# slcs-jsc/jurassic-gpu

Hardware: AMD Instinct MI355X
Metric: rays/s (radiance spectra/s) for limb EGA forward model (higher is better)
Workload: dtype f64; 1 GPU; limb_1e6; rays_total=1000000, channels=4, emitters=5, tables=synthetic 33p x 10T x ~203u per (gas, channel), fp32

## Files before the change

include/jurassic_hip.h:

```cpp
#ifndef JURASSIC_HIP_H
#define JURASSIC_HIP_H

#include "jurassic_abi.h"

#ifdef __cplusplus
extern "C" {
#endif

void formod(ctl_t const *ctl, atm_t *atm, obs_t *obs);
void formod_GPU(ctl_t const *ctl, atm_t *atm, obs_t *obs);
void formod_pencil(ctl_t const *ctl, atm_t *atm, obs_t *obs, int const ir);
void formod_contrib(ctl_t const *ctl, atm_t *atm, obs_t *obs, obs_t *contrib);
void formod_fov(ctl_t const *ctl, obs_t *obs);

void intpol_atm(ctl_t *ctl, atm_t *atm_dest, atm_t *atm_src);

typedef struct { size_t size1, size2, tda; double *data; void *block; int owner; } jur_gsl_matrix_t;
void kernel(ctl_t const *ctl, atm_t *atm, obs_t *obs, jur_gsl_matrix_t *k);

enum {
  JUR_OK = 0,
  JUR_EINVAL = -1,
  JUR_EIO = -2,
  JUR_ENOMEM = -3,
// ... 70 lines not shown
                   int n, double const *dz, double const *w);

int  jur_fov_apply_device(jur_model_t *m, long nr, double const *d_time, double const *d_vpz, double *d_rad,
                          double *d_tau, int n, double const *dz, double const *w, void *stream);

int  jur_intpol_atm(ctl_t const *ctl, atm_t *dest, atm_t const *src, int device);

int  jur_model_reserve(jur_model_t *m, long nr);

long jur_model_workspace_bytes(jur_model_t const *m);
int  jur_model_chunk_rays(jur_model_t const *m);
long jur_model_table_bytes(jur_model_t const *m);
int  jur_device_info(int device, char *pci_bus_id, int len, size_t *free_bytes, size_t *total_bytes);
int  jur_model_set_chunk_rays(jur_model_t *m, int rays);
int  jur_model_set_sort_rays(jur_model_t *m, int on);
int  jur_model_set_trace_multiple(jur_model_t *m, int mult);
int  jur_model_set_compact_workspace(jur_model_t *m, int on);
long jur_model_last_launches(jur_model_t const *m);
int  jur_model_set_workspace_budget(jur_model_t *m, long bytes);

int  jur_model_set_pencil(jur_model_t *m, long max_rays, int rays_per_group);
void jur_tune_trace(int lanes_per_ray);
void jur_tune_combine(int channels_per_group, int sync_segments, long min_lanes);

enum { JUR_ARITH_FAST = 0, JUR_ARITH_EXACT = 1 };
int  jur_model_set_arithmetic(jur_model_t *m, int mode);
int  jur_model_arithmetic(jur_model_t const *m);

int  jur_dropin_finalize(void);

int  jur_model_enable_timing(jur_model_t *m, int on);
int  jur_model_last_kernel_ms(jur_model_t *m, double out_ms[3], long out_launches[3]);
int  jur_model_last_pencil_ms(jur_model_t *m, double *out_ms, long *out_launches);
int  jur_model_last_contrib_ms(jur_model_t *m, double *out_ms, long *out_launches);

int jur_kat_ega_eps(jur_model_t *m, int ig, int id, long n, double const *tau, double const *t, double const *u,
                    double const *p, int mode, int chain, double *out);
int jur_kat_continua(jur_model_t *m, int id, long n, double const *p, double const *t, double const *q,
                     double const *u_co2, double const *u_h2o, double *out);
int jur_kat_update(jur_model_t *m, int id, long n, int what, double const *a, double const *b, double const *c,
                   double *rad, double *tau, double *src);
int jur_kat_traceray(jur_model_t *m, long nr, double const *const geom[7], double *los, double *tsurf, double *const tp[3],
                     int *np_out);

#ifdef __cplusplus
}
// ... 3 lines not shown
```

jurassic-gpu_amd/csrc/jur_internal.h:

```cpp
#ifndef JUR_INTERNAL_H
#define JUR_INTERNAL_H

#include <stdint.h>
#include "jurassic_hip.h"

#ifdef __cplusplus
extern "C" {
#endif

typedef struct { int a, b; } jur_int2;
typedef struct { float u, eps; } jur_ue_t;
typedef struct { float u0, e0, u1, e1; double du_de, de_du; } __attribute__((aligned(32))) jur_rec_t;
typedef struct { double p; int nt; int c0; } jur_lvl_t;
typedef struct { double t; int nu; int e0; } jur_crv_t;

typedef struct {
  double nu;
  double co2_cw296, co2_cw260, co2_cw230;
  double h2o_sc;
  double h2o_ratio;
  double h2o_lnr_hi, h2o_lnr_lo;
  double h2o_ctwfrn;
  double n2_b, n2_beta;
  double o2_b, o2_beta;
// ... 32 lines not shown

typedef struct {
  int n;
  int stride;
  int stride_eps;
  long first;
  int const *order;
  double const *geom[7];
  double *tp[3];
  double *rad, *tau;
  int *np_out;
  int *np;
  double *tsurf;
  double *los;
  double *eps;
  int const *eps_off;
  int *status;
} jur_chunk_t;

int jurk_prepare_atm(jur_view_t const *v, double *d_pslope, void *stream);
int jurk_launch_trace(jur_view_t const *v, jur_chunk_t const *c, void *stream);
int jurk_launch_ega(jur_view_t const *v, jur_chunk_t const *c, void *stream);
int jurk_launch_combine(jur_view_t const *v, jur_chunk_t const *c, void *stream);
int jurk_launch_contrib(jur_view_t const *v, jur_chunk_t const *c, long nr, double *rad_c, double *tau_c, void *stream);
int jurk_tile_max(int n, int const *d_np, int *d_tile_np, void *stream);
int jurk_launch_kquot(long nq, long n, double const *d_rad, double const *d_h, double *d_kq, void *stream);
void jurk_tune_combine(int group, int sync, long min_lanes);
void jurk_tune_trace(int lanes);
int jurk_launch_cg(jur_view_t const *v, jur_chunk_t const *c, double *cgp, double *cgt, double *cgu, void *stream);
int jurk_fill_records(jur_ue_t const *ue, jur_rec_t *rec, long long n, void *stream);
long jurk_sort_tmp_bytes(long nr);
int jurk_sort_rays(jur_view_t const *v, int by_profile, long nr, double const *d_geom, long ld, int *d_order, void *tmp,
                   long tmp_bytes, void *stream);

long jurk_pencil_lds_bytes(jur_view_t const *v, int RB);
int jurk_launch_pencil(jur_view_t const *v, jur_chunk_t const *c, int RB, void *stream);

int jurk_launch_fov(long nr, int nd, double const *time, double const *vpz, double const *rad0, double const *tau0, double *rad,
                    double *tau, long ld, int n, double const *dz, double const *w, int *status, void *stream);

int jurk_launch_intpol(int ip, int ng, int nw, int ns, int nd_, int nx, double cx, double cz, double const *src, double const *x1,
                       int const *idx, int const *nz, double const *dst, double const *x0, double *out, void *stream);

int jurk_kat_ega(jur_view_t const *v, int g, int d, long n, double const *tau, double const *t, double const *u, double const *p,
                 int mode, int chain, double *out, void *stream);
int jurk_kat_continua(jur_view_t const *v, int d, long n, double const *p, double const *t, double const *q, double const *u_co2,
// ... 113 lines not shown
```

jurassic-gpu_amd/csrc/jur_kernels.hip:

```cpp

#include <hip/hip_runtime.h>
#include <hipcub/hipcub.hpp>
#include <cstdlib>
#include <mutex>
#include "jur_internal.h"

#define NLOS JUR_NLOS
#define TBLNS JUR_TBLNS

namespace {

__device__ __forceinline__ double c01(double x) { return (x > 1.) ? 1. : ((x < 0.) ? 0. : x); }
__device__ __forceinline__ double c01_num(double x) { return __builtin_fmax(__builtin_fmin(x, 1.), 0.); }

__device__ __forceinline__ double lip(double x0, double y0, double x1, double y1, double x) {
  return y0 + (x - x0) * (y1 - y0) / (x1 - x0);
}

__device__ __forceinline__ double div_rcp(double a, double b, double r) {
  double const q = a * r;
  return __builtin_fma(__builtin_fma(-b, q, a), r, q);
}
__device__ __forceinline__ double lip_rcp(double x0, double y0, double x1, double y1, double x, double r) {
  return y0 + div_rcp((x - x0) * (y1 - y0), x1 - x0, r);
// ... 1055 lines not shown
  in.p = ldg<double>(row + JUR_F_P * 64, lane);
  in.t = ldg<double>(row + JUR_F_T * 64, lane);
  in.ds = ldg<double>(row + JUR_F_DS * 64, lane);
  in.k = ldg<double>(row + (size_t)f_k * 64, lane);
  in.u_co2 = ldg<double>(row + (size_t)f_co2 * 64, lane);
  in.q_h2o = ldg<double>(row + JUR_F_QH2O * 64, lane);
  in.u_h2o = ldg<double>(row + (size_t)f_h2o * 64, lane);
  double tg[8];
#pragma unroll
  for (int k = 0; k < 8; k++) tg[k] = (k < ng && ((has_table >> k) & 1u)) ? ld_stream(trow + (size_t)k * 64, lane) : 1.0;
  double pcur = 1.0;
#pragma unroll
  for (int k = 0; k < 8; k++) pcur *= tg[k];
  for (int g0 = 8; g0 < ng; g0 += 8) {
#pragma unroll
    for (int k = 0; k < 8; k++) tg[k] = (g0 + k < ng && g0 + k < 32 && ((has_table >> (g0 + k)) & 1u)) ? ld_stream(trow + (size_t)(g0 + k) * 64, lane) : 1.0;
#pragma unroll
    for (int k = 0; k < 8; k++) pcur *= tg[k];
  }
  in.pcur = pcur;
  return in;
}

__global__ __launch_bounds__(256, 6) void jur_combine_kernel(jur_view_t v, jur_chunk_t c, int nrb) {
  int const nd = v.nd, ng = v.ng;
  BlockItem const bi = xcd_block_item((int)blockIdx.x, nrb, nd);
  int const rb = bi.rb, d = bi.item;
  if (rb < 0) return;
  int const r = rb * blockDim.x + threadIdx.x;
  double *const sr = reinterpret_cast<double *>(jur_lds);
  Exp2Lds const e2t{sr + TBLNS};
  {
    double const *const gsr = v.sr + (size_t)d * TBLNS;
    for (int i = threadIdx.x; i < TBLNS; i += blockDim.x) sr[i] = gsr[i];
    if (threadIdx.x < 64) sr[TBLNS + threadIdx.x] = JUR_EXP2_64[threadIdx.x];
    __syncthreads();
  }
  if (r >= c.n) return;
  long const ray = c.order ? (long)c.order[r] : c.first + r;
  int const nfield = JUR_F_K + v.nw + ng;
  int const tile = __builtin_amdgcn_readfirstlane(r >> 6);
  unsigned const lane = (unsigned)(r & 63);
  size_t const R = (size_t)nfield * 64, Re = (size_t)nd * ng * 64;
  double const *const los = c.los + (size_t)tile * los_tile_doubles(nfield);
  double const *const epsb = c.eps + eps_tile_point0(c, tile) * Re + (size_t)d * ng * 64;
  jur_chan_t const ch = v.chan[d];
  int const f_k = JUR_F_K + ch.window, f_u = JUR_F_K + v.nw;
  bool const do_co2 = (v.fourbit & 8) && ch.co2_on, do_h2o = (v.fourbit & 4) && ch.h2o_on,
             do_n2 = (v.fourbit & 2) && ch.n2_on, do_o2 = (v.fourbit & 1) && ch.o2_on;
  size_t const oidx = (size_t)ray * nd + d;
  bool const masked = !isfinite(c.rad[oidx]);
  double rad = 0.0, tau = 1.0, pprev = 1.0;
  int const np = c.np[r];
  unsigned has_table = 0;
  for (int g = 0; g < ng && g < 32; g++) has_table |= (v.pair[g * nd + d].a >= 2 ? 1u : 0u) << g;
  int const f_co2 = do_co2 ? f_u + v.ig_co2 : JUR_F_P, f_h2o = do_h2o ? f_u + v.ig_h2o : JUR_F_P;
  for (int ip = 0; ip < np; ++ip) {
    SegmentIn const in = load_segment(los + (size_t)ip * R, epsb + (size_t)ip * Re, lane, f_k, f_co2, f_h2o, ng, has_table);
    double beta_ds = in.k * in.ds;
    if (do_co2) beta_ds += ctm_co2(ch, in.p, in.t, in.u_co2);
    double const rt = rcp_t(in.t);
    if (do_h2o) beta_ds += ctm_h2o(e2t, ch, in.p, in.t, rt, in.q_h2o, in.u_h2o);
    if (do_n2) beta_ds += ctm_n2(e2t, ch, in.p, in.t, rt) * in.ds;
    if (do_o2) beta_ds += ctm_o2(e2t, ch, in.p, in.t, rt) * in.ds;
    double const tau_gas = segment_tau_gas(in.pcur, pprev);
    pprev = in.pcur;
    new_obs_step(e2t, tau_gas, beta_ds, planck_src(sr, in.t), rad, tau);
  }
  ray_epilogue(sr, ch.nu, c.tsurf[r], v.write_bbt, rad, tau);
  if (masked) rad = __builtin_nan("");
  c.rad[oidx] = rad;
  c.tau[oidx] = tau;
}

#ifndef JUR_COMBINE_WAVES
#define JUR_COMBINE_WAVES 8
#endif
__global__ __launch_bounds__(512, JUR_COMBINE_WAVES) void jur_combine_group_kernel(jur_view_t v, jur_chunk_t c, int nsb, int CG, int SYNC) {
  int const nd = v.nd, ng = v.ng;
  int const ncg = (nd + CG - 1) / CG, SUB = (int)(blockDim.x >> 6) / CG;
  BlockItem const bi = xcd_block_item((int)blockIdx.x, nsb, ncg);
  int const sb = bi.rb, cg = bi.item;
  if (sb < 0) return;
  int const w = __builtin_amdgcn_readfirstlane((int)(threadIdx.x >> 6)), lane = (int)(threadIdx.x & 63);
  int const cw = w % CG, sub = w / CG;
  int const d = cg * CG + cw;
  bool const live_wave = d < nd;
  double *const sr = reinterpret_cast<double *>(jur_lds) + (size_t)cw * TBLNS;
  int *const npmax_sh = reinterpret_cast<int *>(reinterpret_cast<double *>(jur_lds) + (size_t)CG * TBLNS);
  Exp2Lds const e2t{reinterpret_cast<double *>(jur_lds) + (size_t)CG * TBLNS + 2};
  if (threadIdx.x == 0) *npmax_sh = 0;
  if (threadIdx.x < 64) reinterpret_cast<double *>(jur_lds)[(size_t)CG * TBLNS + 2 + threadIdx.x] = JUR_EXP2_64[threadIdx.x];
  for (int k = 0; k < CG; k++) {
    if (cg * CG + k >= nd) break;
    double const *const gsr = v.sr + (size_t)(cg * CG + k) * TBLNS;
// ... 764 lines not shown
  if (c->n <= 0) return 0;
  int const block = 64;
  static int const env_lanes = getenv("JUR_TRACE_LANES") ? atoi(getenv("JUR_TRACE_LANES")) : 0;
  int const forced = g_trace_lanes ? g_trace_lanes : env_lanes;
  int const lanes = forced == 1 || forced == 4 ? forced : ((c->n <= 65536 && v->ng >= 3) ? 4 : 1);
  int const grid = (int)(((long)c->n * lanes + block - 1) / block);
  if (lanes == 4) hipLaunchKernelGGL(jur_trace_lanes_kernel<4>, dim3(grid), dim3(block), 0, (hipStream_t)stream, *v, *c);
  else hipLaunchKernelGGL(jur_trace_kernel, dim3(grid), dim3(block), 0, (hipStream_t)stream, *v, *c);
  return (int)hipGetLastError();
}

static int raise_lds_limit(std::mutex &mu, unsigned long long &raised, void const *const *funcs, int nfunc, bool needed) {
  int dev = 0;
  if (hipGetDevice(&dev) != hipSuccess || dev < 0 || dev > 63) return (int)hipErrorInvalidDevice;
  std::lock_guard<std::mutex> lock(mu);
  if ((raised >> dev) & 1ull) return 0;
  hipError_t e = hipSuccess;
  for (int i = 0; i < nfunc && e == hipSuccess; i++) e = hipFuncSetAttribute(funcs[i], hipFuncAttributeMaxDynamicSharedMemorySize, 128 * 1024);
  if (e != hipSuccess) { (void)hipGetLastError(); return needed ? (int)e : 0; }
  raised |= 1ull << dev;
  return 0;
}

extern "C" int jurk_launch_ega(jur_view_t const *v, jur_chunk_t const *c, void *stream) {
  if (c->n <= 0 || v->ng <= 0) return 0;
  int const block = 256;
  int const nrb = (c->n + block - 1) / block, npair = v->nd * v->ng;
  unsigned const grid = xcd_grid(nrb, npair);
  hipStream_t s = (hipStream_t)stream;
  size_t const lds = (sizeof(jur_lvl_t) + 8) * JUR_TBLNP + (sizeof(jur_crv_t) + 8) * (size_t)v->max_pair_curves;
  bool const use_lds = v->max_pair_curves > 0 && lds <= 48 * 1024;
  bool const rcpb = use_lds && v->fast_arith;
  if (v->sorted_tables) {
    if (rcpb) hipLaunchKernelGGL((jur_ega_kernel<true, true, true>), dim3(grid), dim3(block), lds, s, *v, *c, nrb);
    else if (use_lds) hipLaunchKernelGGL((jur_ega_kernel<true, true, false>), dim3(grid), dim3(block), lds, s, *v, *c, nrb);
    else hipLaunchKernelGGL((jur_ega_kernel<true, false, false>), dim3(grid), dim3(block), 0, s, *v, *c, nrb);
  } else {
    if (use_lds) hipLaunchKernelGGL((jur_ega_kernel<false, true, false>), dim3(grid), dim3(block), lds, s, *v, *c, nrb);
    else hipLaunchKernelGGL((jur_ega_kernel<false, false, false>), dim3(grid), dim3(block), 0, s, *v, *c, nrb);
  }
  return (int)hipGetLastError();
}

static int g_combine_group = -1, g_combine_sync = 8, g_combine_forced = 0;
static long g_combine_min_lanes = 1000000L;
extern "C" void jurk_tune_combine(int group, int sync, long min_lanes) {
  g_combine_forced = group >= 0;
  g_combine_group = group < 0 ? 4 : (group > 6 ? 6 : group);
  g_combine_sync = sync;
  g_combine_min_lanes = min_lanes;
}

extern "C" int jurk_launch_combine(jur_view_t const *v, jur_chunk_t const *c, void *stream) {
  if (c->n <= 0) return 0;
  int const block = 256;
  int const nrb = (c->n + block - 1) / block;
  unsigned const grid = xcd_grid(nrb, v->nd);
  static std::once_flag env_once;
  std::call_once(env_once, [] {
    if (g_combine_group >= 0) return;
    g_combine_group = getenv("JUR_COMBINE_GROUP") ? atoi(getenv("JUR_COMBINE_GROUP")) : 4;
    g_combine_forced = getenv("JUR_COMBINE_GROUP") != NULL;
    if (g_combine_group > 6) g_combine_group = 6;
    if (getenv("JUR_COMBINE_SYNC")) g_combine_sync = atoi(getenv("JUR_COMBINE_SYNC"));
    if (getenv("JUR_COMBINE_MIN_LANES")) g_combine_min_lanes = atol(getenv("JUR_COMBINE_MIN_LANES"));
  });
  if (g_combine_group < 0) g_combine_group = 4;
  int const group = g_combine_group, sync = g_combine_sync;
  bool const fits = g_combine_forced || (group == 4 && (v->nd % 4 == 0 || v->nd >= 64));
  if (group > 0 && v->nd > 1 && fits && (long)c->n * v->nd >= g_combine_min_lanes) {
    int const CG = v->nd < group ? v->nd : group, SUB = 8 / CG, W = CG * SUB;
    int const nsb = (c->n + SUB * 64 - 1) / (SUB * 64), ncg = (v->nd + CG - 1) / CG;
    unsigned const g2 = xcd_grid(nsb, ncg);
    int mask = -1;
    if (sync > 0) { mask = 1; while (mask * 2 <= sync) mask *= 2; mask -= 1; }
    hipLaunchKernelGGL(jur_combine_group_kernel, dim3(g2), dim3(64 * W), sizeof(double) * (JUR_TBLNS * CG + 2 + 64), (hipStream_t)stream,
                       *v, *c, nsb, CG, mask);
    return (int)hipGetLastError();
  }
  hipLaunchKernelGGL(jur_combine_kernel, dim3(grid), dim3(block), sizeof(double) * (JUR_TBLNS + 64), (hipStream_t)stream, *v, *c,
                     nrb);
  return (int)hipGetLastError();
}

extern "C" int jurk_launch_contrib(jur_view_t const *v, jur_chunk_t const *c, long nr, double *rad_c, double *tau_c, void *stream) {
  if (c->n <= 0) return 0;
  int const block = 256;
  int const nrb = (c->n + block - 1) / block;
  long const nitem = (long)v->nd * (v->ng + 1);
  if (((long)(nrb >> 3) + 1) * 8 * nitem * block >= (1L << 32)) return (int)hipErrorInvalidValue;
  unsigned const grid = xcd_grid(nrb, (int)nitem);
  hipLaunchKernelGGL(jur_contrib_kernel, dim3(grid), dim3(block), sizeof(double) * (JUR_TBLNS + 64), (hipStream_t)stream, *v, *c,
                     nrb, nr, rad_c, tau_c);
  return (int)hipGetLastError();
}

extern "C" int jurk_launch_kquot(long nq, long n, double const *d_rad, double const *d_h, double *d_kq, void *stream) {
  if (nq <= 0 || n <= 0) return 0;
  hipLaunchKernelGGL(jur_kquot_kernel, dim3((unsigned)((nq * n + 255) / 256)), dim3(256), 0, (hipStream_t)stream, nq, n, nq, d_rad, d_h, d_kq);
  return (int)hipGetLastError();
}

extern "C" int jurk_tile_max(int n, int const *d_np, int *d_tile_np, void *stream) {
  if (n <= 0) return 0;
// ... 152 lines not shown
```

jurassic-gpu_amd/csrc/jur_model.c:

```c
#define _GNU_SOURCE
#include <math.h>
#include <stdio.h>
#include <stdlib.h>
#include <string.h>
#include <strings.h>
#include <pthread.h>
#include <unistd.h>
#include <sched.h>
#include <hip/hip_runtime_api.h>
#include "jur_internal.h"

#define HIPCHK(call)                                                                       \
  do {                                                                                     \
    hipError_t e_ = (call);                                                                \
    if (e_ != hipSuccess) {                                                                \
      jur_set_error("HIP error %d (%s) at %s:%d", (int)e_, hipGetErrorString(e_), __FILE__, __LINE__); \
      return JUR_EHIP;                                                                     \
    }                                                                                      \
  } while (0)

struct jur_model {
  int device;
  int shared_tables;
  ctl_t *ctl;
  jur_view_t view;
  long table_bytes;
  void *d_chan, *d_sr, *d_pair, *d_pair_e0, *d_lvl, *d_crv, *d_ue, *d_rec;
  int arith;
  void *d_atm;
  int atm_cap;
  int atm_slices;
  double atm_zmin, atm_zmax;
  int chunk_rays;
  int nfield;
  double *d_los;
  double *d_eps;
  long ws_budget;
  long ws_rays;
  long ws_trace_rays;
  int trace_mult;
  long use_rays, use_trace_rays;
  int *d_np;
  double *d_tsurf;
  int compact_ws;
  int use_compact;
  int *d_tile_np, *d_eps_off;
  int *h_tile;
  long n_launch_ega;
  int *d_status;
  long los_bytes;
  int sort_rays;
  int *d_order;
  void *d_sort_tmp;
  long order_cap, sort_tmp_bytes;
  double *d_io;
  int *d_io_np;
  long io_cap;
  int *h_status;
  double *h_io;
  long h_io_cap;
  double *h_pkg;
  double *h_atm;
  long h_atm_n, h_atm_cap;
  double h_atm_hydz;
  hipStream_t stream;
  hipStream_t stream2;
  hipEvent_t ev_mask, ev_trace;
  int host_call;
  hipEvent_t ev_done;
// ... 360 lines not shown
    return JUR_OK;
  }
  if ((long)(nrow * n) > m->h_atm_cap) {
    free(m->h_atm);
    m->h_atm = (double *)malloc(sizeof(double) * nrow * n);
    m->h_atm_cap = m->h_atm ? (long)(nrow * n) : 0;
  }
  m->h_atm_n = 0;
  if (m->h_atm) { memcpy(m->h_atm, h, sizeof(double) * nrow * n); m->h_atm_n = n; m->h_atm_hydz = m->ctl->hydz; }
  hydrostatic_rows(m, h, (size_t)n, 0, n);
  int const rc = upload_atm_rows(m, h, n);
  if (rc) m->h_atm_n = 0;
  free(h);
  return rc;
}

static void free_workspace(jur_model_t *m) {
  if (m->d_los) (void)hipFree(m->d_los);
  if (m->d_eps) (void)hipFree(m->d_eps);
  if (m->d_np) (void)hipFree(m->d_np);
  if (m->d_tsurf) (void)hipFree(m->d_tsurf);
  if (m->d_tile_np) (void)hipFree(m->d_tile_np);
  if (m->d_eps_off) (void)hipFree(m->d_eps_off);
  if (m->h_tile) (void)hipHostFree(m->h_tile);
  m->d_los = NULL; m->d_eps = NULL; m->d_np = NULL; m->d_tsurf = NULL; m->d_tile_np = NULL; m->d_eps_off = NULL; m->h_tile = NULL;
  m->los_bytes = 0; m->ws_rays = 0; m->ws_trace_rays = 0;
}

static int ensure_workspace(jur_model_t *m, long nr) {
  long const per_ray_los = (long)sizeof(double) * m->nfield * JUR_NLOS;
  long const per_ray_eps = (long)sizeof(double) * m->view.nd * (m->view.ng > 0 ? m->view.ng : 1) * JUR_NLOS;
  long budget = m->ws_budget;
  int asked = 0;
  for (int attempt = 0;; attempt++) {
    long R = m->chunk_rays;
    long const fit = budget / (per_ray_los + per_ray_eps);
    if (R > fit) R = fit / 64 * 64;
    if (R < 64) R = 64;
    if (nr <= R) R = (nr + 63) / 64 * 64;
    else {
      long const nchunk = (nr + R - 1) / R;
      R = ((nr + nchunk - 1) / nchunk + 63) / 64 * 64;
    }
    long mult = m->trace_mult > 0 ? m->trace_mult : 1;
    while (mult > 1 && (per_ray_los * mult + per_ray_eps) * R > budget) mult--;
    long Rt = R * mult;
    if (nr < Rt) Rt = (nr + R - 1) / R * R;
    int compact = 0;
// ... 5 lines not shown
      if (R_c >= 64 && Rt_c >= R_c) { R = R_c; Rt = Rt_c; compact = 1; }
    }
    if (R <= m->ws_rays && Rt <= m->ws_trace_rays) {
      m->use_rays = R;
      m->use_trace_rays = Rt;
      m->use_compact = compact;
      return JUR_OK;
    }
    if (!asked) {
      size_t free_b = 0, total_b = 0;
      asked = 1;
      if (hipMemGetInfo(&free_b, &total_b) == hipSuccess) {
        long const avail = (long)free_b + m->los_bytes - (2L << 30);
        if (avail > (64L << 20) && avail < budget) { budget = avail; continue; }
      } else (void)hipGetLastError();
    }
    free_workspace(m);
    hipError_t e = hipMalloc((void **)&m->d_los, (size_t)per_ray_los * Rt);
    if (e == hipSuccess) e = hipMalloc((void **)&m->d_eps, (size_t)per_ray_eps * R);
    if (e == hipSuccess) e = hipMalloc((void **)&m->d_np, sizeof(int) * Rt);
    if (e == hipSuccess) e = hipMalloc((void **)&m->d_tsurf, sizeof(double) * Rt);
    if (e == hipSuccess) e = hipMalloc((void **)&m->d_tile_np, sizeof(int) * (Rt / 64 + 1));
    if (e == hipSuccess) e = hipMalloc((void **)&m->d_eps_off, sizeof(int) * (Rt / 64 + 1));
    if (e == hipSuccess) e = hipHostMalloc((void **)&m->h_tile, sizeof(int) * 2 * (Rt / 64 + 1), hipHostMallocDefault);
    if (e == hipSuccess) {
      m->los_bytes = per_ray_los * Rt + per_ray_eps * R;
      m->ws_rays = R;
      m->ws_trace_rays = Rt;
      m->use_rays = R;
      m->use_trace_rays = Rt;
      m->use_compact = compact;
      return JUR_OK;
    }
    (void)hipGetLastError();
    free_workspace(m);
    if (R <= 64 || attempt >= 24) {
      jur_set_error("cannot allocate the workspace (%ld B per ray, even for %ld rays): %s", per_ray_los + per_ray_eps, R,
                    hipGetErrorString(e));
      return JUR_EHIP;
    }
    budget = (per_ray_los + per_ray_eps) * R / 2;
  }
}

long jur_model_workspace_bytes(jur_model_t const *m) { return m->los_bytes; }
long jur_model_table_bytes(jur_model_t const *m) { return m->table_bytes; }
// ... 31 lines not shown
int jur_model_set_trace_multiple(jur_model_t *m, int mult) {
  if (mult < 1 || mult > 64) { jur_set_error("trace multiple must be in 1..64"); return JUR_EINVAL; }
  m->trace_mult = mult;
  return JUR_OK;
}

int jur_model_set_chunk_rays(jur_model_t *m, int rays) {
  if (rays < 64 || rays > (1 << 22)) { jur_set_error("chunk_rays must be in 64..4194304"); return JUR_EINVAL; }
  m->chunk_rays = (rays + 63) / 64 * 64;
  return JUR_OK;
}

int jur_model_set_pencil(jur_model_t *m, long max_rays, int rays_per_group) {
  if (max_rays < 0 || rays_per_group < 0 || rays_per_group > 64) { jur_set_error("set_pencil: max_rays >= 0, rays_per_group in 0..64"); return JUR_EINVAL; }
  m->pencil_rays = max_rays;
  m->pencil_rb = rays_per_group;
  return JUR_OK;
}

void jur_tune_trace(int lanes_per_ray) { jurk_tune_trace(lanes_per_ray); }

void jur_tune_combine(int channels_per_group, int sync_segments, long min_lanes) {
  jurk_tune_combine(channels_per_group, sync_segments, min_lanes);
}

int jur_model_enable_timing(jur_model_t *m, int on) {
  HIPCHK(hipSetDevice(m->device));
  if (on && !m->evpool) {
    m->evpool = (hipEvent_t *)calloc(2 * JUR_MAX_TIMED, sizeof(hipEvent_t));
    m->evkind = (unsigned char *)calloc(JUR_MAX_TIMED, 1);
    if (!m->evpool || !m->evkind) return JUR_ENOMEM;
    for (int i = 0; i < 2 * JUR_MAX_TIMED; i++) HIPCHK(hipEventCreate(&m->evpool[i]));
  }
  m->timing = on;
  m->ntimed = 0;
  return JUR_OK;
}

int jur_model_last_kernel_ms(jur_model_t *m, double out_ms[3], long out_launches[3]) {
  for (int k = 0; k < 3; k++) { out_ms[k] = 0; out_launches[k] = 0; }
  if (!m->evpool) return JUR_OK;
  HIPCHK(hipSetDevice(m->device));
  for (int i = 0; i < m->ntimed; i++) {
    float ms = 0;
    HIPCHK(hipEventSynchronize(m->evpool[2 * i + 1]));
    HIPCHK(hipEventElapsedTime(&ms, m->evpool[2 * i], m->evpool[2 * i + 1]));
// ... 132 lines not shown
    return record_done(m, s);
  }
  rc = ensure_workspace(m, nr);
  if (rc) return rc;
  long const R = m->use_rays;
  int const *order = NULL;
  if (m->sort_rays && nr > 64) {
    rc = ensure_sort_buffers(m, nr);
    if (rc) return rc;
    int const by_profile = m->atm_slices > 1 && nr >= 1024L * m->atm_slices;
    int const e = jurk_sort_rays(&m->view, by_profile, nr, d_geom, ldg, m->d_order, m->d_sort_tmp, m->sort_tmp_bytes, s);
    if (e) { jur_set_error("ray sort failed: %s", hipGetErrorString((hipError_t)e)); return JUR_EHIP; }
    order = m->d_order;
  }
  long const Rt = m->use_trace_rays;
  m->n_launch_ega = 0;
#define TIMED(kind, launch, what)                                                              \
  do {                                                                                         \
    int const ti_ = (m->timing && m->ntimed < JUR_MAX_TIMED) ? m->ntimed++ : -1;               \
    if (ti_ >= 0) { m->evkind[ti_] = (kind); HIPCHK(hipEventRecord(m->evpool[2 * ti_], s)); } \
    int const e_ = (launch);                                                                   \
    if (e_) { jur_set_error(what " kernel launch failed: %s", hipGetErrorString((hipError_t)e_)); return JUR_EHIP; } \
    if (ti_ >= 0) HIPCHK(hipEventRecord(m->evpool[2 * ti_ + 1], s));                          \
  } while (0)
  for (long t0 = 0; t0 < nr; t0 += Rt) {
    jur_chunk_t c;
    long const nt = (nr - t0 < Rt) ? nr - t0 : Rt;
    c.stride = (int)Rt;
    c.stride_eps = (int)R;
    for (int k = 0; k < 7; k++) c.geom[k] = d_geom + (size_t)k * ldg;
    for (int k = 0; k < 3; k++) c.tp[k] = d_tp + (size_t)k * ldtp;
    c.rad = d_rad;
    c.tau = d_tau;
    c.np_out = d_np;
    c.eps = m->d_eps;
    c.status = d_status ? d_status : m->d_status;
    c.n = (int)nt;
    c.first = t0;
    c.order = order ? order + t0 : NULL;
    c.np = m->d_np;
    c.tsurf = m->d_tsurf;
    c.los = m->d_los;
    TIMED(0, jurk_launch_trace(&m->view, &c, s), "trace");
    if (m->host_call) {
      if (t0 == 0) HIPCHK(hipStreamWaitEvent(s, m->ev_mask, 0));
      if (t0 + Rt >= nr) HIPCHK(hipEventRecord(m->ev_trace, s));
// ... 16 lines not shown
      for (long t = 0; t < ntile; t++) total += h_np[t];
      long const nchunk = (total + cap - 1) / cap > 0 ? (total + cap - 1) / cap : 1;
      long const target = (total + nchunk - 1) / nchunk;
      for (long t = 0; t < ntile;) {
        long acc = 0, e = t;
        while (e < ntile && (e == t || (acc + h_np[e] <= cap && acc < target))) acc += h_np[e++];
        if (e < ntile && e - t >= 64) e = t + (e - t) / 32 * 32;
        acc = 0;
        for (long q = t; q < e; q++) { h_off[q] = (int)acc; acc += h_np[q]; h_np[q] = (q == t); }
        t = e;
      }
      HIPCHK(hipMemcpyAsync(m->d_eps_off, h_off, sizeof(int) * ntile, hipMemcpyHostToDevice, s));
      for (long t0c = 0; t0c < ntile;) {
        long t1c = t0c + 1;
        while (t1c < ntile && !h_np[t1c]) t1c++;
        long const s0 = t0c * 64, s1 = (t1c * 64 < nt) ? t1c * 64 : nt;
        c.n = (int)(s1 - s0);
        c.first = t0 + s0;
        c.order = order ? order + t0 + s0 : NULL;
        c.np = m->d_np + s0;
        c.tsurf = m->d_tsurf + s0;
        c.los = m->d_los + (size_t)s0 * JUR_NLOS * m->nfield;
        c.eps_off = m->d_eps_off + t0c;
        TIMED(1, jurk_launch_ega(&m->view, &c, s), "ega");
        if (co) TIMED(4, jurk_launch_contrib(&m->view, &c, nr, co->rad, co->tau, s), "contribution");
        TIMED(2, jurk_launch_combine(&m->view, &c, s), "combine");
        m->n_launch_ega++;
        t0c = t1c;
      }
      continue;
    }
    for (long s0 = 0; s0 < nt; s0 += R) {
      c.n = (int)((nt - s0 < R) ? nt - s0 : R);
      c.first = t0 + s0;
      c.order = order ? order + t0 + s0 : NULL;
      c.np = m->d_np + s0;
      c.tsurf = m->d_tsurf + s0;
      c.los = m->d_los + (size_t)s0 * JUR_NLOS * m->nfield;
      TIMED(1, jurk_launch_ega(&m->view, &c, s), "ega");
      if (co) TIMED(4, jurk_launch_contrib(&m->view, &c, nr, co->rad, co->tau, s), "contribution");
      TIMED(2, jurk_launch_combine(&m->view, &c, s), "combine");
      m->n_launch_ega++;
    }
  }
#undef TIMED
  return record_done(m, s);
}

void *jur_host_alloc(size_t bytes) {
  void *p = NULL;
  if (hipHostMalloc(&p, bytes ? bytes : 8, hipHostMallocDefault) != hipSuccess) {
    (void)hipGetLastError();
    jur_set_error("hipHostMalloc of %zu bytes failed", bytes);
    return NULL;
  }
  return p;
}
void jur_host_free(void *p) { if (p) (void)hipHostFree(p); }

static int is_pinned(void const *p) {
  hipPointerAttribute_t a;
  if (!p) return 0;
  if (hipPointerGetAttributes(&a, p) != hipSuccess) { (void)hipGetLastError(); return 0; }
  return a.type == hipMemoryTypeHost;
}

typedef struct { char *dst; char const *src; size_t n; } cpjob_t;
// ... 1131 lines not shown
```

jurassic-gpu_amd/jurassic_hip/lib.py:

```python
import ctypes as C
import os
import numpy as np
from . import abi

PKG = os.path.dirname(os.path.dirname(os.path.abspath(__file__)))
SO = os.environ.get("JURASSIC_HIP_SO",
                    os.path.join(PKG, "libjurassic_hip%s.so" % os.environ.get("JUR_SUFFIX", "")))
_lib = None
dp = C.POINTER(C.c_double)


class JurassicError(RuntimeError):
    pass


def lib():
    global _lib
    if _lib is None:
        if not os.path.exists(SO):
            raise JurassicError(f"{SO} not built: run `make -C jurassic-gpu_amd/csrc` "
                                "or __graft_entry__.build(); no CPU fallback exists")
        L = C.CDLL(SO)
        L.jur_last_error.restype = C.c_char_p
        L.jur_fov_read_shape.argtypes = [C.c_char_p, C.POINTER(C.c_int), dp, dp]
# ... 43 lines not shown
        L.jur_model_last_launches.argtypes = [C.c_void_p]
        L.jur_model_set_compact_workspace.argtypes = [C.c_void_p, C.c_int]
        L.jur_model_set_chunk_rays.argtypes = [C.c_void_p, C.c_int]
        L.jur_model_set_sort_rays.argtypes = [C.c_void_p, C.c_int]
        L.jur_model_set_trace_multiple.argtypes = [C.c_void_p, C.c_int]
        L.jur_model_set_workspace_budget.argtypes = [C.c_void_p, C.c_long]
        L.jur_model_enable_timing.argtypes = [C.c_void_p, C.c_int]
        L.jur_model_last_kernel_ms.argtypes = [C.c_void_p, dp, C.POINTER(C.c_long)]
        L.jur_model_last_pencil_ms.argtypes = [C.c_void_p, dp, C.POINTER(C.c_long)]
        L.jur_model_last_contrib_ms.argtypes = [C.c_void_p, dp, C.POINTER(C.c_long)]
        L.jur_model_set_pencil.argtypes = [C.c_void_p, C.c_long, C.c_int]
        L.jur_model_set_arithmetic.argtypes = [C.c_void_p, C.c_int]
        L.jur_model_arithmetic.argtypes = [C.c_void_p]
        L.jur_multi_balance.argtypes = [C.c_void_p, C.c_long, C.POINTER(dp), C.c_int, C.POINTER(C.c_long)]
        L.jur_estimate_los_points.argtypes = [C.c_double] * 4 + [C.c_long, C.POINTER(dp), dp]
        L.jur_balance_rays.argtypes = [C.c_double] * 4 + [C.c_long, C.POINTER(dp), C.c_int, C.POINTER(C.c_long)]
        L.jur_models_set_atm.argtypes = [C.POINTER(C.c_void_p), C.c_int, C.c_void_p]
        L.jur_formod_host_multi.argtypes = [C.POINTER(C.c_void_p), C.c_int, C.c_long, C.POINTER(dp), dp, dp, C.POINTER(dp), C.POINTER(C.c_int)]
        L.jur_formod_device_multi.argtypes = [C.POINTER(C.c_void_p), C.c_int, C.c_long, C.POINTER(C.c_long)] + [C.c_void_p] * 7
        L.jur_tune_combine.argtypes = [C.c_int, C.c_int, C.c_long]
        L.jur_tune_combine.restype = None
        L.jur_tune_trace.argtypes = [C.c_int]
        L.jur_tune_trace.restype = None
        L.jur_state_size.restype = C.c_size_t
        L.jur_state_size.argtypes = [C.c_void_p, C.c_void_p]
        L.jur_measurement_size.restype = C.c_size_t
        L.jur_measurement_size.argtypes = [C.c_void_p, C.c_void_p]
        L.jur_kernel.argtypes = [C.c_void_p, C.c_void_p, C.c_void_p, dp, C.c_size_t, C.c_size_t]
        ip_, lp_ = C.POINTER(C.c_int), C.POINTER(C.c_long)
        L.jur_scene_layout.argtypes = [C.c_void_p, C.c_void_p, C.c_long, dp, ip_, ip_, lp_]
        L.jur_scene_columns.restype = C.c_long
        L.jur_scene_columns.argtypes = [C.c_void_p, C.c_void_p, C.c_int, C.c_int, lp_]
        L.jur_kernel_scene_host.argtypes = [C.c_void_p, C.c_void_p, C.c_long, C.POINTER(dp), dp, dp, C.POINTER(dp), ip_, lp_, dp,
                                            C.c_long]
        L.jur_model_last_scene_ms.argtypes = [C.c_void_p, dp, lp_]
        L.jur_abi_sizes.argtypes = [C.POINTER(C.c_size_t)]
        L.jur_kat_ega_eps.argtypes = [C.c_void_p, C.c_int, C.c_int, C.c_long, dp, dp, dp, dp, C.c_int, C.c_int, dp]
        L.jur_kat_continua.argtypes = [C.c_void_p, C.c_int, C.c_long] + [dp] * 6
        L.jur_kat_update.argtypes = [C.c_void_p, C.c_int, C.c_long, C.c_int] + [dp] * 6
        L.jur_kat_traceray.argtypes = [C.c_void_p, C.c_long, C.POINTER(dp), dp, dp, C.POINTER(dp), C.POINTER(C.c_int)]
        for name in ("formod", "formod_GPU"):
            getattr(L, name).argtypes = [C.c_void_p] * 3
            getattr(L, name).restype = None
        L.kernel.argtypes = [C.c_void_p] * 4
        L.kernel.restype = None
        L.formod_pencil.argtypes = [C.c_void_p] * 3 + [C.c_int]
# ... 452 lines not shown
    dz, w = np.zeros(abi.NSHAPE), np.zeros(abi.NSHAPE)
    n = C.c_int(0)
    _chk(lib().jur_fov_read_shape(path.encode(), C.byref(n), _p(dz), _p(w)))
    return dz[:n.value].copy(), w[:n.value].copy()


def fov_apply(time, vpz, rad, tau, dz, w):
    time, vpz, dz, w = (np.ascontiguousarray(a, dtype=np.float64) for a in (time, vpz, dz, w))
    assert rad.flags.c_contiguous and tau.flags.c_contiguous and rad.dtype == np.float64 and rad.shape == tau.shape
    nr, nd = rad.shape
    _chk(lib().jur_fov_apply(nd, nr, _p(time), _p(vpz), _p(rad), _p(tau), nd, len(dz), _p(dz), _p(w)))


def formod_pencil(ctl, atm, obs, ir):
    lib().formod_pencil(C.byref(ctl), C.byref(atm), C.byref(obs), ir)


def tune_trace(lanes_per_ray=0):
    lib().jur_tune_trace(lanes_per_ray)


def tune_combine(channels_per_group=4, sync_segments=8, min_lanes=1_000_000):
    lib().jur_tune_combine(channels_per_group, sync_segments, min_lanes)
```

Measured before the change: 18.96 million rays/s.

## Fuse EGA emissivity and combine kernels via last-arriving-block atomic counter

Adds a fused kernel that computes per-(channel, gas) EGA path transmittances. The last block to finish all gases for a ray block and channel, detected with an atomic arrival counter and release/acquire fences, then performs the radiance combine step. This removes the separate combine launch and its tail/launch gap, overlapping combine work with remaining EGA blocks. It costs a per-chunk memset of the counters, fences, and tighter launch bounds. It falls back to separate kernels when contributions are requested or tables are not in the strict fast layout.

New measurement: 13.29 million rays/s. -29.9%, worse.

```diff
diff --git a/include/jurassic_hip.h b/include/jurassic_hip.h
--- a/include/jurassic_hip.h
+++ b/include/jurassic_hip.h
@@ -116,6 +116,8 @@
 int  jur_model_set_pencil(jur_model_t *m, long max_rays, int rays_per_group);
 void jur_tune_trace(int lanes_per_ray);
 void jur_tune_combine(int channels_per_group, int sync_segments, long min_lanes);
+void jur_tune_update_fusion(int mode);
+int  jur_update_fusion_rule(int strict_tables, int contributions, long rays, int nd, int ng);
 
 enum { JUR_ARITH_FAST = 0, JUR_ARITH_EXACT = 1 };
 int  jur_model_set_arithmetic(jur_model_t *m, int mode);
diff --git a/jurassic-gpu_amd/csrc/jur_internal.h b/jurassic-gpu_amd/csrc/jur_internal.h
--- a/jurassic-gpu_amd/csrc/jur_internal.h
+++ b/jurassic-gpu_amd/csrc/jur_internal.h
@@ -78,6 +78,11 @@
 int jurk_launch_trace(jur_view_t const *v, jur_chunk_t const *c, void *stream);
 int jurk_launch_ega(jur_view_t const *v, jur_chunk_t const *c, void *stream);
 int jurk_launch_combine(jur_view_t const *v, jur_chunk_t const *c, void *stream);
+int jurk_launch_ega_update(jur_view_t const *v, jur_chunk_t const *c, int *arrive, void *stream);
+int jurk_ega_update_applies(jur_view_t const *v, jur_chunk_t const *c, int contrib);
+int jurk_update_fusion_rule(int strict, int contrib, long rays, int nd, int ng);
+long jurk_arrive_bytes(jur_view_t const *v, long n);
+void jurk_tune_update_fusion(int mode);
 int jurk_launch_contrib(jur_view_t const *v, jur_chunk_t const *c, long nr, double *rad_c, double *tau_c, void *stream);
 int jurk_tile_max(int n, int const *d_np, int *d_tile_np, void *stream);
 int jurk_launch_kquot(long nq, long n, double const *d_rad, double const *d_h, double *d_kq, void *stream);
diff --git a/jurassic-gpu_amd/csrc/jur_kernels.hip b/jurassic-gpu_amd/csrc/jur_kernels.hip
--- a/jurassic-gpu_amd/csrc/jur_kernels.hip
+++ b/jurassic-gpu_amd/csrc/jur_kernels.hip
@@ -1101,21 +1101,16 @@
   return in;
 }
 
-__global__ __launch_bounds__(256, 6) void jur_combine_kernel(jur_view_t v, jur_chunk_t c, int nrb) {
+__device__ __forceinline__ void stage_source(jur_view_t const &v, int d, double *sr) {
+  double const *const gsr = v.sr + (size_t)d * TBLNS;
+  for (int i = threadIdx.x; i < TBLNS; i += blockDim.x) sr[i] = gsr[i];
+  if (threadIdx.x < 64) sr[TBLNS + threadIdx.x] = JUR_EXP2_64[threadIdx.x];
+  __syncthreads();
+}
+
+__device__ __forceinline__ void combine_lane(jur_view_t const &v, jur_chunk_t const &c, int d, int r, double const *sr,
+                                             Exp2Lds const e2t) {
   int const nd = v.nd, ng = v.ng;
-  BlockItem const bi = xcd_block_item((int)blockIdx.x, nrb, nd);
-  int const rb = bi.rb, d = bi.item;
-  if (rb < 0) return;
-  int const r = rb * blockDim.x + threadIdx.x;
-  double *const sr = reinterpret_cast<double *>(jur_lds);
-  Exp2Lds const e2t{sr + TBLNS};
-  {
-    double const *const gsr = v.sr + (size_t)d * TBLNS;
-    for (int i = threadIdx.x; i < TBLNS; i += blockDim.x) sr[i] = gsr[i];
-    if (threadIdx.x < 64) sr[TBLNS + threadIdx.x] = JUR_EXP2_64[threadIdx.x];
-    __syncthreads();
-  }
-  if (r >= c.n) return;
   long const ray = c.order ? (long)c.order[r] : c.first + r;
   int const nfield = JUR_F_K + v.nw + ng;
   int const tile = __builtin_amdgcn_readfirstlane(r >> 6);
@@ -1123,7 +1118,8 @@
   size_t const R = (size_t)nfield * 64, Re = (size_t)nd * ng * 64;
   double const *const los = c.los + (size_t)tile * los_tile_doubles(nfield);
   double const *const epsb = c.eps + eps_tile_point0(c, tile) * Re + (size_t)d * ng * 64;
-  jur_chan_t const ch = v.chan[d];
+  typedef unsigned chan_words_t __attribute__((ext_vector_type(sizeof(jur_chan_t) / 4)));
+  jur_chan_t const ch = __builtin_bit_cast(jur_chan_t, ld_scalar<chan_words_t>(v.chan, (unsigned)d * (unsigned)sizeof(jur_chan_t)));
   int const f_k = JUR_F_K + ch.window, f_u = JUR_F_K + v.nw;
   bool const do_co2 = (v.fourbit & 8) && ch.co2_on, do_h2o = (v.fourbit & 4) && ch.h2o_on,
              do_n2 = (v.fourbit & 2) && ch.n2_on, do_o2 = (v.fourbit & 1) && ch.o2_on;
@@ -1150,6 +1146,88 @@
   if (masked) rad = __builtin_nan("");
   c.rad[oidx] = rad;
   c.tau[oidx] = tau;
+}
+
+__global__ __launch_bounds__(256, 6) void jur_combine_kernel(jur_view_t v, jur_chunk_t c, int nrb) {
+  BlockItem const bi = xcd_block_item((int)blockIdx.x, nrb, v.nd);
+  int const rb = bi.rb, d = bi.item;
+  if (rb < 0) return;
+  int const r = rb * blockDim.x + threadIdx.x;
+  double *const sr = reinterpret_cast<double *>(jur_lds);
+  stage_source(v, d, sr);
+  if (r >= c.n) return;
+  combine_lane(v, c, d, r, sr, Exp2Lds{sr + TBLNS});
+}
+
+__global__ __launch_bounds__(256, 8) void jur_ega_update_kernel(jur_view_t v, jur_chunk_t c, int nrb, int *__restrict__ arrive) {
+  int const npair = v.nd * v.ng;
+  BlockItem const bi = xcd_block_item((int)blockIdx.x, nrb, npair);
+  int const rb = bi.rb, pr = bi.item;
+  if (rb < 0) return;
+  int const d = pr / v.ng, g = pr - d * v.ng;
+  int const tile = rb * 4 + __builtin_amdgcn_readfirstlane((int)(threadIdx.x >> 6));
+  unsigned const lane = (unsigned)(threadIdx.x & 63);
+  int const r = tile * 64 + (int)lane;
+  int const pair_idx = g * v.nd + d;
+  jur_int2 const pd = v.pair[pair_idx];
+  if (pd.a >= 2) {
+    PairDesc<true> D{v.lvl, v.crv, v.ue + v.pair_e0[pair_idx], (unsigned)pd.b, 0u, 0u, 0u};
+    D.recb = v.rec + v.pair_e0[pair_idx];
+    stage_pair<true, true>(v, pd, D);
+    if (r < c.n) {
+      int const nfield = JUR_F_K + v.nw + v.ng;
+      size_t const R = (size_t)nfield * 64;
+      double const *const los_tile = c.los + (size_t)tile * los_tile_doubles(nfield);
+      double const *const los_p = los_tile + JUR_F_P * 64, *const los_t = los_tile + JUR_F_T * 64,
+                   *const los_u = los_tile + (size_t)(JUR_F_K + v.nw + g) * 64;
+      size_t const Re = (size_t)npair * 64;
+      double *const out = c.eps + eps_tile_point0(c, tile) * Re + (size_t)pr * 64;
+      int const np = c.np[r];
+      double tau_path = 1.0;
+      unsigned br = 0, ia = 0, ib = 0;
+      double p_next = 0., t_next = 0.;
+      if (np > 0) { p_next = ldg<double>(los_p, lane); t_next = ldg<double>(los_t, lane); }
+      for (int ip = 0; ip < np; ++ip) {
+        size_t const o = (size_t)ip * R;
+        double const p = p_next, t = t_next;
+        if (ip + 1 < np) { p_next = ldg<double>(los_p + o + R, lane); t_next = ldg<double>(los_t + o + R, lane); }
+        double const u = ldg<double>(los_u + o, lane);
+        tau_path = ega_eps_warm<true, true, true>(v, pd, D, tau_path, t, u, p, br, ia, ib);
+#ifdef JUR_FUSE_SC1
+        __hip_atomic_store(reinterpret_cast<double *>(reinterpret_cast<char *>(out + (size_t)ip * Re) + (size_t)(lane * 8u)), tau_path,
+                           __ATOMIC_RELAXED, __HIP_MEMORY_SCOPE_AGENT);
+#else
+        st_stream(out + (size_t)ip * Re, lane, tau_path);
+#endif
+      }
+    }
+  }
+  int *const last_sh = reinterpret_cast<int *>(jur_lds);
+  asm volatile("s_waitcnt vmcnt(0)" ::: "memory");
+  __syncthreads();
+  bool const lane0 = tile == rb * 4 && lane == 0;
+  if (lane0) {
+#ifndef JUR_FUSE_SC1
+    __builtin_amdgcn_fence(__ATOMIC_RELEASE, "agent");
+    asm volatile("s_waitcnt vmcnt(0)" ::: "memory");
+#endif
+    int const before = __hip_atomic_fetch_add(&arrive[rb * v.nd + d], 1, __ATOMIC_RELAXED, __HIP_MEMORY_SCOPE_AGENT);
+    *last_sh = (before == v.ng - 1);
+  }
+  __syncthreads();
+#ifdef JUR_FUSE_NOCONT
+  if (true) return;
+#endif
+  if (!__builtin_amdgcn_readfirstlane(*last_sh)) return;
+  if (lane0) {
+    __builtin_amdgcn_fence(__ATOMIC_ACQUIRE, "agent");
+    asm volatile("s_waitcnt vmcnt(0)" ::: "memory");
+  }
+  __syncthreads();
+  double *const sr = reinterpret_cast<double *>(jur_lds);
+  stage_source(v, d, sr);
+  if (r >= c.n) return;
+  combine_lane(v, c, d, r, sr, Exp2Lds{sr + TBLNS});
 }
 
 #ifndef JUR_COMBINE_WAVES
@@ -1960,14 +2038,19 @@
   return 0;
 }
 
+static size_t ega_lds_bytes(jur_view_t const *v) {
+  return (sizeof(jur_lvl_t) + 8) * JUR_TBLNP + (sizeof(jur_crv_t) + 8) * (size_t)v->max_pair_curves;
+}
+static bool ega_use_lds(jur_view_t const *v) { return v->max_pair_curves > 0 && ega_lds_bytes(v) <= 48 * 1024; }
+
 extern "C" int jurk_launch_ega(jur_view_t const *v, jur_chunk_t const *c, void *stream) {
   if (c->n <= 0 || v->ng <= 0) return 0;
   int const block = 256;
   int const nrb = (c->n + block - 1) / block, npair = v->nd * v->ng;
   unsigned const grid = xcd_grid(nrb, npair);
   hipStream_t s = (hipStream_t)stream;
-  size_t const lds = (sizeof(jur_lvl_t) + 8) * JUR_TBLNP + (sizeof(jur_crv_t) + 8) * (size_t)v->max_pair_curves;
-  bool const use_lds = v->max_pair_curves > 0 && lds <= 48 * 1024;
+  size_t const lds = ega_lds_bytes(v);
+  bool const use_lds = ega_use_lds(v);
   bool const rcpb = use_lds && v->fast_arith;
   if (v->sorted_tables) {
     if (rcpb) hipLaunchKernelGGL((jur_ega_kernel<true, true, true>), dim3(grid), dim3(block), lds, s, *v, *c, nrb);
@@ -1989,11 +2072,7 @@
   g_combine_min_lanes = min_lanes;
 }
 
-extern "C" int jurk_launch_combine(jur_view_t const *v, jur_chunk_t const *c, void *stream) {
-  if (c->n <= 0) return 0;
-  int const block = 256;
-  int const nrb = (c->n + block - 1) / block;
-  unsigned const grid = xcd_grid(nrb, v->nd);
+static void combine_env() {
   static std::once_flag env_once;
   std::call_once(env_once, [] {
     if (g_combine_group >= 0) return;
@@ -2003,6 +2082,14 @@
     if (getenv("JUR_COMBINE_SYNC")) g_combine_sync = atoi(getenv("JUR_COMBINE_SYNC"));
     if (getenv("JUR_COMBINE_MIN_LANES")) g_combine_min_lanes = atol(getenv("JUR_COMBINE_MIN_LANES"));
   });
+}
+
+extern "C" int jurk_launch_combine(jur_view_t const *v, jur_chunk_t const *c, void *stream) {
+  if (c->n <= 0) return 0;
+  int const block = 256;
+  int const nrb = (c->n + block - 1) / block;
+  unsigned const grid = xcd_grid(nrb, v->nd);
+  combine_env();
   if (g_combine_group < 0) g_combine_group = 4;
   int const group = g_combine_group, sync = g_combine_sync;
   bool const fits = g_combine_forced || (group == 4 && (v->nd % 4 == 0 || v->nd >= 64));
@@ -2018,6 +2105,38 @@
   }
   hipLaunchKernelGGL(jur_combine_kernel, dim3(grid), dim3(block), sizeof(double) * (JUR_TBLNS + 64), (hipStream_t)stream, *v, *c,
                      nrb);
+  return (int)hipGetLastError();
+}
+
+static int g_update_fusion = 0, g_update_fusion_set = 0;
+extern "C" void jurk_tune_update_fusion(int mode) { g_update_fusion = mode > 0 ? 1 : 0; g_update_fusion_set = mode >= 0; }
+
+extern "C" int jurk_update_fusion_rule(int strict, int contrib, long rays, int nd, int ng) {
+  static int const env_mode = getenv("JUR_UPDATE_FUSION") ? atoi(getenv("JUR_UPDATE_FUSION")) : -1;
+  combine_env();
+  int const mode = g_update_fusion_set ? g_update_fusion : (env_mode < 0 ? -1 : (env_mode > 0 ? 1 : 0));
+  if (mode == 0 || !strict || contrib || g_combine_forced || rays <= 0 || nd <= 0 || ng <= 0) return 0;
+  return mode == 1 || rays * nd >= g_combine_min_lanes;
+}
+extern "C" int jurk_ega_update_applies(jur_view_t const *v, jur_chunk_t const *c, int contrib) {
+  bool const strict = v->sorted_tables && ega_use_lds(v) && v->fast_arith && v->rec != NULL;
+  return jurk_update_fusion_rule(strict, contrib, c->n, v->nd, v->ng);
+}
+extern "C" long jurk_arrive_bytes(jur_view_t const *v, long n) {
+  return (((n + 255) / 256 * (long)v->nd * (long)sizeof(int)) + 15) / 16 * 16;
+}
+
+extern "C" int jurk_launch_ega_update(jur_view_t const *v, jur_chunk_t const *c, int *arrive, void *stream) {
+  if (c->n <= 0 || v->ng <= 0) return 0;
+  if (!jurk_ega_update_applies(v, c, 0) || !arrive) return (int)hipErrorInvalidValue;
+  int const block = 256;
+  int const nrb = (c->n + block - 1) / block, npair = v->nd * v->ng;
+  unsigned const grid = xcd_grid(nrb, npair);
+  hipStream_t s = (hipStream_t)stream;
+  size_t const lds_ega = ega_lds_bytes(v), lds_upd = sizeof(double) * (JUR_TBLNS + 64);
+  hipError_t const e = hipMemsetAsync(arrive, 0, (size_t)jurk_arrive_bytes(v, c->n), s);
+  if (e != hipSuccess) return (int)e;
+  hipLaunchKernelGGL(jur_ega_update_kernel, dim3(grid), dim3(block), lds_ega > lds_upd ? lds_ega : lds_upd, s, *v, *c, nrb, arrive);
   return (int)hipGetLastError();
 }
 
diff --git a/jurassic-gpu_amd/csrc/jur_model.c b/jurassic-gpu_amd/csrc/jur_model.c
--- a/jurassic-gpu_amd/csrc/jur_model.c
+++ b/jurassic-gpu_amd/csrc/jur_model.c
@@ -45,6 +45,7 @@
   int compact_ws;
   int use_compact;
   int *d_tile_np, *d_eps_off;
+  int *d_arrive;
   int *h_tile;
   long n_launch_ega;
   int *d_status;
@@ -451,8 +452,10 @@
   if (m->d_tsurf) (void)hipFree(m->d_tsurf);
   if (m->d_tile_np) (void)hipFree(m->d_tile_np);
   if (m->d_eps_off) (void)hipFree(m->d_eps_off);
+  if (m->d_arrive) (void)hipFree(m->d_arrive);
   if (m->h_tile) (void)hipHostFree(m->h_tile);
   m->d_los = NULL; m->d_eps = NULL; m->d_np = NULL; m->d_tsurf = NULL; m->d_tile_np = NULL; m->d_eps_off = NULL; m->h_tile = NULL;
+  m->d_arrive = NULL;
   m->los_bytes = 0; m->ws_rays = 0; m->ws_trace_rays = 0;
 }
 
@@ -504,6 +507,7 @@
     if (e == hipSuccess) e = hipMalloc((void **)&m->d_tsurf, sizeof(double) * Rt);
     if (e == hipSuccess) e = hipMalloc((void **)&m->d_tile_np, sizeof(int) * (Rt / 64 + 1));
     if (e == hipSuccess) e = hipMalloc((void **)&m->d_eps_off, sizeof(int) * (Rt / 64 + 1));
+    if (e == hipSuccess) e = hipMalloc((void **)&m->d_arrive, (size_t)jurk_arrive_bytes(&m->view, Rt));
     if (e == hipSuccess) e = hipHostMalloc((void **)&m->h_tile, sizeof(int) * 2 * (Rt / 64 + 1), hipHostMallocDefault);
     if (e == hipSuccess) {
       m->los_bytes = per_ray_los * Rt + per_ray_eps * R;
@@ -581,6 +585,11 @@
 
 void jur_tune_combine(int channels_per_group, int sync_segments, long min_lanes) {
   jurk_tune_combine(channels_per_group, sync_segments, min_lanes);
+}
+
+void jur_tune_update_fusion(int mode) { jurk_tune_update_fusion(mode); }
+int jur_update_fusion_rule(int strict_tables, int contributions, long rays, int nd, int ng) {
+  return jurk_update_fusion_rule(strict_tables, contributions, rays, nd, ng);
 }
 
 int jur_model_enable_timing(jur_model_t *m, int on) {
@@ -759,6 +768,16 @@
     int const e_ = (launch);                                                                   \
     if (e_) { jur_set_error(what " kernel launch failed: %s", hipGetErrorString((hipError_t)e_)); return JUR_EHIP; } \
     if (ti_ >= 0) HIPCHK(hipEventRecord(m->evpool[2 * ti_ + 1], s));                          \
+  } while (0)
+#define INTEGRATE()                                                                                        \
+  do {                                                                                                     \
+    if (jurk_ega_update_applies(&m->view, &c, co != NULL))                                                 \
+      TIMED(1, jurk_launch_ega_update(&m->view, &c, m->d_arrive, s), "ega + update");                    \
+    else {                                                                                                 \
+      TIMED(1, jurk_launch_ega(&m->view, &c, s), "ega");                                                  \
+      if (co) TIMED(4, jurk_launch_contrib(&m->view, &c, nr, co->rad, co->tau, s), "contribution");       \
+      TIMED(2, jurk_launch_combine(&m->view, &c, s), "combine");                                          \
+    }                                                                                                      \
   } while (0)
   for (long t0 = 0; t0 < nr; t0 += Rt) {
     jur_chunk_t c;
@@ -821,9 +840,7 @@
         c.tsurf = m->d_tsurf + s0;
         c.los = m->d_los + (size_t)s0 * JUR_NLOS * m->nfield;
         c.eps_off = m->d_eps_off + t0c;
-        TIMED(1, jurk_launch_ega(&m->view, &c, s), "ega");
-        if (co) TIMED(4, jurk_launch_contrib(&m->view, &c, nr, co->rad, co->tau, s), "contribution");
-        TIMED(2, jurk_launch_combine(&m->view, &c, s), "combine");
+        INTEGRATE();
         m->n_launch_ega++;
         t0c = t1c;
       }
@@ -836,12 +853,11 @@
       c.np = m->d_np + s0;
       c.tsurf = m->d_tsurf + s0;
       c.los = m->d_los + (size_t)s0 * JUR_NLOS * m->nfield;
-      TIMED(1, jurk_launch_ega(&m->view, &c, s), "ega");
-      if (co) TIMED(4, jurk_launch_contrib(&m->view, &c, nr, co->rad, co->tau, s), "contribution");
-      TIMED(2, jurk_launch_combine(&m->view, &c, s), "combine");
+      INTEGRATE();
       m->n_launch_ega++;
     }
   }
+#undef INTEGRATE
 #undef TIMED
   return record_done(m, s);
 }
diff --git a/jurassic-gpu_amd/jurassic_hip/lib.py b/jurassic-gpu_amd/jurassic_hip/lib.py
--- a/jurassic-gpu_amd/jurassic_hip/lib.py
+++ b/jurassic-gpu_amd/jurassic_hip/lib.py
@@ -89,6 +89,10 @@
         L.jur_tune_combine.restype = None
         L.jur_tune_trace.argtypes = [C.c_int]
         L.jur_tune_trace.restype = None
+        L.jur_tune_update_fusion.argtypes = [C.c_int]
+        L.jur_tune_update_fusion.restype = None
+        L.jur_update_fusion_rule.argtypes = [C.c_int, C.c_int, C.c_long, C.c_int, C.c_int]
+        L.jur_update_fusion_rule.restype = C.c_int
         L.jur_state_size.restype = C.c_size_t
         L.jur_state_size.argtypes = [C.c_void_p, C.c_void_p]
         L.jur_measurement_size.restype = C.c_size_t
@@ -587,3 +591,11 @@
 
 def tune_combine(channels_per_group=4, sync_segments=8, min_lanes=1_000_000):
     lib().jur_tune_combine(channels_per_group, sync_segments, min_lanes)
+
+
+def tune_update_fusion(mode=-1):
+    lib().jur_tune_update_fusion(mode)
+
+
+def update_fusion_rule(strict_tables, contributions, rays, nd, ng):
+    return bool(lib().jur_update_fusion_rule(int(strict_tables), int(contributions), rays, nd, ng))
```
